# zhenghao2519/Beyond-Fixed-Forms

Measured on AMD Instinct MI355X. Metric: scenes/sec (2D->3D projection+refinement), 200k pts x 300 views, higher is better.
Workload: dtype f64

## Files before the change

beyond_fixed_forms_amd/_lib.py:

```python
from __future__ import annotations

import ctypes
import os
import time
from ctypes import c_double, c_float, c_int32, c_int64, c_void_p

import torch

_HERE = os.path.dirname(os.path.abspath(__file__))
LIB_PATH = os.environ.get("BFF_HIP_LIB") or os.path.join(_HERE, "lib", "libbff_hip.so")
CSRC_DIR = os.path.join(_HERE, "csrc")

_P, _I, _L, _D, _F = c_void_p, c_int32, c_int64, c_double, c_float

SIGNATURES = {
    "bff_rle_to_maskbits": [_P, _P, _P, _P, _I, _L, _I, _P, _P, _P],
    "bff_rle_to_labels": [_P, _P, _P, _P, _I, _L, _I, _P, _P, _P, _P],
    "bff_mask_row_directory": [_P, _P, _P, _I, _I, _I, _P, _P],
    "bff_project_views_lookup": [_P, _L, _L, _P, _P, _I, _P, _I, _I, _I, _P, _I, _I, _D, _P, _P, _P, _P, _P, _I, _P, _P, _P, _P, _P, _L, _L, _P, _P, _P, _P],
    "bff_project_views_cached": [_L, _I, _P, _I, _I, _P, _P, _P, _P, _P, _P, _P, _P, _I, _P, _P, _P, _P, _P, _L, _L, _P, _P, _P, _P],
    "bff_visibility_table": [_P, _L, _L, _P, _P, _I, _P, _I, _I, _I, _I, _I, _D, _P, _P, _P, _P, _L, _P, _I, _P],
    "bff_masks2d_count": [_P, _I, _L, _P, _P, _P],
    "bff_masks2d_runs": [_P, _I, _L, _P, _P, _P, _P],
    "bff_project_views": [_P, _L, _L, _P, _P, _I, _P, _P, _I, _I, _D, _P, _P, _P, _I, _P, _P, _P, _P, _P, _L, _L, _P, _P, _P, _P, _P],
    "bff_depth_tile_u16": [_P, _I, _I, _I, _P, _I, _P],
    "bff_project_views_u16": [_P, _L, _L, _P, _P, _I, _P, _I, _I, _I, _P, _I, _I, _D, _P, _P, _P, _I, _P, _P, _P, _P, _P, _L, _L, _P, _P, _P, _P, _P],
    "bff_point_tile_bounds": [_P, _L, _L, _P, _P],
    "bff_count_viewed": [_P, _L, _L, _P, _P, _I, _P, _I, _I, _I, _P, _I, _I, _D, _I, _P, _P, _P],
    "bff_render_depth_u16": [_P, _L, _L, _P, _P, _I, _I, _I, _I, _I, _I, _P, _P, _P, _P],
    "bff_render_splat_depth_u16": [_P, _L, _L, _P, _P, _I, _I, _I, _I, _I, _D, _I, _P, _P, _P, _P],
    "bff_point_labels": [_P, _I, _L, _L, _P, _P, _P],
    "bff_render_labels_u16": [_P, _L, _L, _P, _P, _P, _I, _I, _I, _I, _I, _D, _I, _P, _P, _P, _P, _P],
    "bff_label_runs_count": [_P, _I, _I, _I, _I, _I, _I, _P, _P, _P],
    "bff_label_runs_emit": [_P, _I, _I, _I, _I, _I, _I, _P, _L, _P, _P, _P, _P],
    "bff_render_mesh_depth_u16": [_P, _L, _L, _P, _L, _P, _P, _I, _I, _I, _I, _I, _I, _P, _P, _P],
    "bff_render_mesh_depth_clip_u16": [_P, _L, _L, _P, _L, _P, _P, _I, _I, _I, _I, _I, _D, _I, _P, _P, _P],
# ... 59 lines not shown
    "bff_dbscan_elements": [_P, _I, _L, _L, _P, _P, _P, _P, _P],
    "bff_dbscan_core": [_P, _I, _L, _P, _L, _P, _P, _P, _P, _L, _L, _P, _D, _D, _I, _P, _P],
    "bff_dbscan_link": [_P, _P, _P, _P, _I, _L, _P, _L, _P, _P, _P, _P, _L, _L, _P, _D, _D, _I, _P, _P],
}
PLAIN = {"bff_abi_version": (c_int32, []), "bff_last_error": (ctypes.c_char_p, []), "bff_arch": (ctypes.c_char_p, []),
         "bff_masks2d_tile_pixels": (c_int32, []), "bff_label_runs_tile_pixels": (c_int32, []), "bff_mask_lookup_rows": (c_int32, [c_int32, c_int32, c_int64]),
         "bff_cosine_gemm_path": (c_int32, [c_int32, c_int32, c_int32]),
         "bff_cross_popcount_slices": (c_int32, [c_int32, c_int32, c_int64]),
         "bff_chunk_mask_words": (c_int32, [c_int64]), "bff_label_plane_stride": (c_int64, [c_int64]), "bff_resolve_overlaps_max_rows": (c_int32, []),
         "bff_point_tile_size": (c_int32, []), "bff_sweep_frames_per_block": (c_int32, [c_int64, c_int32]), "bff_mesh_lane_box": (c_int32, []), "bff_splat_lane_box": (c_int32, []), "bff_depth_tiled_texels": (c_int64, [c_int32, c_int32]), "bff_merge_scratch_words": (c_int64, [c_int32]), "bff_merge_uses_chunk_bound": (c_int32, [c_int64]),
         "bff_profile_next_merge": (c_int32, [_P, _P]), "bff_group_slice_cap": (c_int32, [c_int32, c_int32]),
         "bff_point_threshold_scratch_words": (c_int64, [c_int64]), "bff_point_threshold_capacity": (c_int32, []), "bff_point_threshold_capacity_set": (c_int32, [c_int32]), "bff_scene_header_words": (c_int32, [c_int32, c_int32]), "bff_scene_struct_bytes": (c_int32, [c_int32]),
         "bff_host_component_csr": (c_int32, [_P, _P, _I, _I, _P, _P, _P, _P]),
         "bff_visibility_words": (c_int64, [c_int64]), "bff_visibility_builds": (c_int64, []),
         "bff_visibility_table_bytes": (c_int32, [c_int64, c_int32, c_int64, _P]),
         "bff_profile_next_sweep": (c_int32, [_P, _P]), "bff_event_create": (c_void_p, []),
         "bff_event_destroy": (c_int32, [_P]), "bff_event_elapsed_ms": (c_int32, [_P, _P, _P]),
         "bff_event_record": (c_int32, [_P, _P]), "bff_event_synchronize": (c_int32, [_P])}
ABI_VERSION = 16


class BffLibraryError(RuntimeError):
    pass


_lib = None


def load():
    global _lib
# ... 225 lines not shown


def visibility_builds():
    return int(load().bff_visibility_builds())


def visibility_table_bytes(n_points, n_slots, n_pixels=0):
    out = (c_int64 * 3)()
    rc = load().bff_visibility_table_bytes(n_points, n_slots, n_pixels, ctypes.cast(out, c_void_p))
    if rc != 0:
        raise RuntimeError(f"bff_visibility_table_bytes failed ({rc}): {load().bff_last_error().decode()}")
    return tuple(int(v) for v in out)


def visibility_table(xyz_soa, n_points, slot_inv_pose, cam_intr, depth, height, width, depth_thresh, tile_bounds=None,
                     depth_size=None, max_bytes=None):
    dev = xyz_soa.device
    n_slots = int(slot_inv_pose.shape[0])
    stride = visibility_words(n_points)
    hs, ws, layout = _depth_layout(depth, depth_size)
    if max_bytes is not None and sum(visibility_table_bytes(n_points, n_slots)) > max_bytes:
        return None
    mask = torch.empty((n_slots, stride), dtype=i64, device=dev)
    off = torch.empty((n_slots, stride), dtype=i32, device=dev)
    total = torch.zeros(1, dtype=i64, device=dev)
    head = (_ptr(xyz_soa, f64), n_points, xyz_soa.shape[1], _ptr(slot_inv_pose, f64), _k9(cam_intr), n_slots, _ptr(depth),
            hs, ws, layout, height, width, float(depth_thresh), _ptr(tile_bounds, f64), _ptr(mask, i64), _ptr(off, i32))
    call("bff_visibility_table", *head, None, 0, _ptr(total, i64), 1)
    n_pixels = int(total.item())
    if n_pixels >= 1 << 32 or (max_bytes is not None and sum(visibility_table_bytes(n_points, n_slots, n_pixels)) > max_bytes):
        return None
    pix = torch.empty(max(n_pixels, 1), dtype=i32, device=dev)
    call("bff_visibility_table", *head, _ptr(pix, i32), n_pixels, _ptr(total, i64), 2)
    return mask, off, pix


def project_views_cached(n_points, depth_index, height, width, vis, mask_tab, mask_dir, run_start, run_end, view_mask_offs,
                         word_bits, frame_mask, frame_rowbase, frame_nmask, frame_flags, rows, masked_count, viewed_count,
                         chunk_mask=None):
    call("bff_project_views_cached", n_points, depth_index.shape[0], _ptr(depth_index, i32), height, width,
         _ptr(vis[0], i64), _ptr(vis[1], i32), _ptr(vis[2], i32), _ptr(mask_tab, i32), _ptr(mask_dir, i32),
         _ptr(run_start, i32), _ptr(run_end, i32), _ptr(view_mask_offs, i32), word_bits, _ptr(frame_mask, i32),
         _ptr(frame_rowbase, i32), _ptr(frame_nmask, i32), _ptr(frame_flags, i32), _ptr(rows, i64),
         0 if rows is None else rows.shape[0], (n_points + 63) // 64, _ptr(chunk_mask, i64), _ptr(masked_count, i32),
         _ptr(viewed_count, i32))


def count_viewed(xyz_soa, n_points, inv_pose, cam_intr, depth, depth_index, height, width, depth_thresh, viewed_count,
                 tile_bounds=None, depth_size=None, frames_per_block=None):
    k = (c_double * 9)(*[float(v) for v in cam_intr.reshape(-1)])
    if depth.dtype == torch.int16 or depth_size is not None:
        hs, ws = (depth_size if depth_size is not None else depth.shape[1:3])
        layout = 0 if depth_size is None else (2 if depth.dtype == f32 else 1)
    else:
        hs, ws, layout = 0, 0, -1
        if depth.dtype != f32:
            raise TypeError(f"expected float32 depth images, got {depth.dtype}")
    if frames_per_block is None:
# ... 570 lines not shown
```

beyond_fixed_forms_amd/csrc/project.hip:

```cpp
#include <hip/hip_ext.h>

#include "common.h"
#include "mask_rows.h"

namespace bff {

constexpr int kBlock = 256;
constexpr int kPPT = 4;
constexpr int kWordsPerBlock = (kBlock / kWave) * kPPT;
constexpr int kPtsPerBlock = kWordsPerBlock * kWave;

struct Intrinsics { double k[9]; };

struct RawDepth {
    const uint32_t *taps;
    int n_taps;
    int texel_f32;
    int64_t frame_stride;
    float scale;
};

struct VisTable {
    const uint64_t *mask;
    const uint32_t *off;
// ... 728 lines not shown
    const int slot = blockIdx.y;
    if (w >= stride) return;
    const uint64_t m = mask[slot * stride + w];
    if (!((m >> lane) & 1)) return;
    const int64_t n = w * kWave + lane;
    const double px = xyz[n], py = xyz[n_pad + n], pz = xyz[2 * n_pad + n];
    const double *P = inv_pose + 16 * (int64_t)slot;
    const double cx = fma(P[3], 1.0, fma(P[2], pz, fma(P[1], py, fma(P[0], px, 0.0))));
    const double cy = fma(P[7], 1.0, fma(P[6], pz, fma(P[5], py, fma(P[4], px, 0.0))));
    const double cz = fma(P[11], 1.0, fma(P[10], pz, fma(P[9], py, fma(P[8], px, 0.0))));
    const double p0 = fma(K.k[2], cz, fma(K.k[1], cy, fma(K.k[0], cx, 0.0)));
    const double p1 = fma(K.k[5], cz, fma(K.k[4], cy, fma(K.k[3], cx, 0.0)));
    const double u = rint(p0 / cz), v = rint(p1 / cz);
    const int64_t at = (int64_t)off[slot * stride + w] + __popcll(m & ((1ull << lane) - 1));
    if (at < pix_cap) pixels[at] = (uint32_t)(int)u | ((uint32_t)(int)v << 16);
}

constexpr int kWaveChunk = 1024;
constexpr int kPx = kWaveChunk / kWave;
constexpr int kWaveChunks = 16384 / kWaveChunk;

__device__ __forceinline__ int chunk_word_slot(int i) { return i ^ ((((i >> 5) & 3) | ((i >> 4) & 8)) << 2); }

__device__ __forceinline__ uint32_t wave_xor_scan(uint32_t v)
{
#define BFF_DPP_XOR(ctrl, rows) v ^= (uint32_t)__builtin_amdgcn_update_dpp(0, (int)v, ctrl, rows, 0xF, false)
    BFF_DPP_XOR(0x111, 0xF);
    BFF_DPP_XOR(0x112, 0xF);
    BFF_DPP_XOR(0x114, 0xF);
    BFF_DPP_XOR(0x118, 0xF);
// ... 582 lines not shown
                                        int32_t word_bits, const int32_t *frame_mask, const int32_t *frame_rowbase,
                                        const int32_t *frame_nmask, const int32_t *frame_flags, uint64_t *rows, int64_t n_rows,
                                        int64_t nw, uint64_t *chunk_mask, int32_t *masked_count, int32_t *viewed_count,
                                        void *stream)
{
    if (n_points <= 0 || n_frames <= 0) return BFF_OK;
    BFF_REQUIRE(height > 0 && width > 0, "bff_project_views_cached: bad image size");
    BFF_REQUIRE(vis_mask && vis_off && vis_pix, "bff_project_views_cached: null table");
    const MaskRows mr{reinterpret_cast<const uint4 *>(mask_tab), mask_dir, run_start, run_end, view_mask_offs};
    const VisTable vt{vis_mask, vis_off, vis_pix, bff_visibility_words(n_points)};
    return project_views_launch(nullptr, n_points, n_points, nullptr, nullptr, n_frames, nullptr, nullptr, depth_index, height,
                                width, 0.0, nullptr, nullptr, nullptr, word_bits, frame_mask, frame_rowbase, frame_nmask,
                                frame_flags, rows, n_rows, nw, chunk_mask, masked_count, viewed_count, nullptr, stream, &mr, &vt);
}

extern "C" int64_t bff_visibility_words(int64_t n_points)
{
    return n_points <= 0 ? 0 : ceil_div(n_points, (int64_t)kPtsPerBlock) * kWordsPerBlock;
}

extern "C" int bff_visibility_table_bytes(int64_t n_points, int32_t n_slots, int64_t n_pixels, int64_t *bytes)
{
    BFF_REQUIRE(n_points >= 0 && n_slots >= 0 && n_pixels >= 0 && bytes, "bff_visibility_table_bytes: bad arguments");
    const int64_t entries = bff_visibility_words(n_points) * n_slots;
    bytes[0] = (int64_t)sizeof(uint64_t) * entries;
    bytes[1] = (int64_t)sizeof(uint32_t) * entries;
    bytes[2] = (int64_t)sizeof(uint32_t) * n_pixels;
    return BFF_OK;
}

// ... 124 lines not shown
```

beyond_fixed_forms_amd/csrc/scene.hip:

```cpp
#include "rows.h"

using namespace bff;

namespace {

__global__ void order_keys_kernel(const int64_t *__restrict__ sig, const int32_t *__restrict__ label_id, int n,
                                  int sig_bits, int64_t *__restrict__ keys)
{
    const int i = blockIdx.x * blockDim.x + threadIdx.x;
    if (i < n) keys[i] = ((int64_t)label_id[i] << sig_bits) | sig[i];
}

int bits_for(int n)
{
    int b = 1;
    while ((1 << b) < n && b < 31) ++b;
    return b;
}

}

#define BFF_TRY(call) do { const int rc_ = (call); if (rc_ != BFF_OK) return rc_; } while (0)

extern "C" int32_t bff_scene_header_words(int32_t s1_rows, int32_t cap)
// ... 53 lines not shown
    struct Prezeroed {
        Prezeroed() { scratch_prezeroed() = 1; }
        ~Prezeroed() { scratch_prezeroed() = 0; }
    } prezeroed_scope;
    void *hv = (ws->heavy_stream && ws->heavy_stream != stream) ? ws->heavy_stream : stream;
    const bool two = hv != stream;
    auto hand_over = [&](void *event, void *from, void *to) -> int {
        hipError_t ee = hipEventRecord(reinterpret_cast<hipEvent_t>(event), as_stream(from));
        if (ee == hipSuccess) ee = hipStreamWaitEvent(as_stream(to), reinterpret_cast<hipEvent_t>(event), 0);
        return ee == hipSuccess ? BFF_OK : fail((int)ee, "bff_scene_project: stream hand-over: %s", hipGetErrorString(ee));
    };
    if (two) {
        BFF_REQUIRE(ws->events[0] && ws->events[1] && ws->events[2] && ws->events[3], "bff_scene_project: a heavy stream needs the workspace's four events");
        BFF_TRY(hand_over(ws->events[0], stream, hv));
    }
    if (lookup) {
        BFF_REQUIRE(ws->mask_tab && ws->mask_dir, "bff_scene_project: no row directory buffers");
        BFF_TRY(bff_mask_row_directory(sc->run_start, sc->run_end, sc->mask_run_offs, n_rows, sc->height, sc->width,
                                       ws->mask_tab, ws->mask_dir, hv));
    } else {
        BFF_TRY(bff_rle_to_labels(sc->run_start, sc->run_end, sc->mask_run_offs, sc->view_mask_offs, sc->n_mviews, hw,
                                  sc->word_bits, ws->labels, ws->maskbits, ws->segmap, hv));
    }
    const bool ratio = pr->filter_mode == 2;
    int32_t *const sweep_viewed = (ratio && !viewed_in) ? ws->viewed : nullptr;
    const int32_t *const viewed = ratio ? (viewed_in ? viewed_in : ws->viewed) : nullptr;
    if (lookup && sc->vis_mask && sc->vis_off && sc->vis_pix)
        BFF_TRY(bff_project_views_cached(n, sc->n_frames, sc->depth_index, sc->height, sc->width, sc->vis_mask, sc->vis_off,
                                         sc->vis_pix, ws->mask_tab, ws->mask_dir, sc->run_start, sc->run_end,
                                         sc->view_mask_offs, sc->word_bits, sc->frame_mask, sc->frame_rowbase, sc->frame_nmask,
                                         sc->frame_flags, ws->rows, n_rows, nw, ws->chunk_mask, ws->masked, sweep_viewed, hv));
    else if (lookup)
        BFF_TRY(bff_project_views_lookup(sc->xyz, n, sc->n_pad, sc->inv_pose, sc->cam_intr, sc->n_frames,
                                         sc->depth_raw ? sc->depth_raw : (const void *)sc->depth, sc->depth_h, sc->depth_w,
                                         sc->depth_raw ? sc->depth_tiled : -1, sc->depth_index, sc->height, sc->width,
                                         pr->depth_thresh, ws->mask_tab, ws->mask_dir, sc->run_start, sc->run_end,
                                         sc->view_mask_offs, sc->word_bits, sc->frame_mask, sc->frame_rowbase, sc->frame_nmask,
                                         sc->frame_flags, ws->rows, n_rows, nw, ws->chunk_mask, ws->masked, sweep_viewed,
                                         sc->tile_bounds, hv));
    else if (sc->depth_raw)
        BFF_TRY(bff_project_views_u16(sc->xyz, n, sc->n_pad, sc->inv_pose, sc->cam_intr, sc->n_frames, sc->depth_raw,
                                      sc->depth_h, sc->depth_w, sc->depth_tiled, sc->depth_index, sc->height, sc->width, pr->depth_thresh,
// ... 87 lines not shown
```

beyond_fixed_forms_amd/pipeline.py:

```python
from __future__ import annotations

import ctypes
import os
import time
from ctypes import c_double, c_float, c_int32, c_int64, c_size_t, c_void_p

import numpy as np
import torch

from . import _lib

GROUP_CAP = 256
GROUP_CAP_MAX = 512
HDR_K, HDR_NUNIQUE, HDR_THR, HDR_OVERFLOW = 0, 4, 5, 6


def hdr_offsets(cap):
    return tuple(16 + k * cap for k in range(6))


class SceneStruct(ctypes.Structure):
    _fields_ = [("n_points", c_int64), ("n_pad", c_int64), ("nw", c_int64),
                ("xyz", c_void_p), ("tile_bounds", c_void_p), ("inv_pose", c_void_p), ("cam_intr", c_double * 9),
                ("depth", c_void_p), ("depth_raw", c_void_p),
                ("depth_index", c_void_p), ("frame_mask", c_void_p), ("frame_rowbase", c_void_p),
                ("frame_nmask", c_void_p), ("frame_flags", c_void_p),
                ("run_start", c_void_p), ("run_end", c_void_p), ("mask_run_offs", c_void_p), ("view_mask_offs", c_void_p),
                ("conf", c_void_p), ("label_id", c_void_p), ("unsort", c_void_p), ("perm", c_void_p),
                ("s1_run_start", c_void_p), ("s1_run_end", c_void_p), ("s1_row_run_offs", c_void_p),
                ("height", c_int32), ("width", c_int32), ("n_frames", c_int32), ("n_mviews", c_int32),
                ("word_bits", c_int32), ("n_rows", c_int32), ("conf_f16", c_int32), ("n_label_ids", c_int32),
                ("s1_rows", c_int32), ("depth_h", c_int32), ("depth_w", c_int32), ("depth_tiled", c_int32),
                ("vis_mask", c_void_p), ("vis_off", c_void_p), ("vis_pix", c_void_p)]


class ParamsStruct(ctypes.Structure):
    _fields_ = [("depth_thresh", c_double), ("filter_fraction", c_double), ("iou_thres", c_float),
                ("min_members", c_int32), ("filter_mode", c_int32), ("filter_sort", c_int32)]


_WS_PTRS = ["maskbits", "segmap", "labels", "rows", "chunk_mask", "keep", "tile_mask", "agg", "both",
            "masked", "viewed", "sel_scratch", "area", "mean_word", "order", "parent", "comp", "count",
            "gmembers", "goffs", "slices", "pair_scratch", "vals", "vals_sorted", "hist", "merge_scratch", "chunk_pop",
            "sig", "sig_keys", "sig_sorted", "sort_temp", "mask_tab", "mask_dir"]


class WorkspaceStruct(ctypes.Structure):
    _fields_ = [(n, c_void_p) for n in _WS_PTRS] + [("sort_temp_bytes", c_size_t), ("zero_bytes", c_size_t),
# ... 71 lines not shown
        setattr(s, k, _p(getattr(ds, k)))
    s.conf, s.unsort, s.perm = _p(ds.conf), _p(ds.unsort), _p(ds.perm)
    if ds.unsort is not None and ds.perm is None:
        raise ValueError("a spatially sorted scene needs its inverse permutation (DeviceScene.perm)")
    s.height, s.width = ds.height, ds.width
    s.n_frames = ds.n_frames if n_frames is None else n_frames
    s.n_mviews = ds.view_mask_offs.shape[0] - 1
    s.word_bits, s.n_rows = ds.word_bits, ds.n_rows
    s.conf_f16 = 1 if ds.conf.dtype == torch.float16 else 0
    s.n_label_ids = ds.n_label_ids
    if stage1 is not None:
        s.s1_run_start, s.s1_run_end, s.s1_row_run_offs = _p(stage1.run_start), _p(stage1.run_end), _p(stage1.row_run_offs)
        s.s1_rows = stage1.row_run_offs.shape[0] - 1
    if vis is not None:
        s.vis_mask, s.vis_off, s.vis_pix = _p(vis.mask), _p(vis.off), _p(vis.pix)
    return s


def params_struct(cfg, depth_thresh, filter_sort=False):
    _check_layout()
    p = ParamsStruct()
    from .scene import with_viewed_counts
    p.filter_sort = 1 if filter_sort else 0
    ratio = with_viewed_counts(cfg)
    p.depth_thresh = float(depth_thresh)
    p.filter_mode = 1 if cfg.if_occurance_threshold else (2 if ratio else 0)
    p.filter_fraction = float(cfg.detected_ratio_threshold if ratio else cfg.occurance_threshold)
    p.iou_thres = float(cfg.iou_thres)
    p.min_members = int(cfg.min_aggragated_masks)
    return p
# ... 309 lines not shown
```

beyond_fixed_forms_amd/projection.py:

```python
from __future__ import annotations

import dataclasses
from typing import List, Optional

import numpy as np
import torch

import os

from . import _lib, pipeline
from .scene import (DEPTH_THRESH, DeviceScene, prepare_class, prepare_geometry, prepare_scene,
                    with_viewed_counts)
from .timing import merge_span, span, sweep_span


@dataclasses.dataclass
class Stage2Result:
    scene_id: str
    n_points: int
    rows: torch.Tensor
    conf: torch.Tensor
    final_class: List[str]
    groups: list
    debug: dict
# ... 123 lines not shown
    stage1: Optional[object] = None


def fast_path_ok(ds: DeviceScene) -> bool:
    return (ds.n_rows > 0 and ds.n_points > 0 and ds.view_mask_offs.shape[0] > 1 and ds.n_mask_frames > 0
            and ds.xyz.is_cuda and os.environ.get("BFF_NO_FAST") != "1")


@dataclasses.dataclass
class VisibilityTable:
    mask: torch.Tensor
    off: torch.Tensor
    pix: torch.Tensor
    ready: torch.cuda.Event
    streams: set


def vis_table_max_bytes():
    return int(float(os.environ.get("BFF_VIS_TABLE_MAX_MB", "512")) * (1 << 20))


def scene_visibility(ds: DeviceScene, depth_thresh) -> Optional[VisibilityTable]:
    if os.environ.get("BFF_VIS_TABLE", "1") == "0" or not _lib.mask_lookup_rows(ds.height, ds.width, ds.n_rows):
        return None
    owner = ds.geometry if ds.geometry is not None else ds
    tables = owner.__dict__.setdefault("_vis_tables", {})
    key = float(depth_thresh)
    tab = tables.get(key)
    if tab is None:
        tables[key] = "visited"
        return None
    if tab is False:
        return None
    raw = _lib.raw_stream()
    if tab == "visited":
        dev = ds.xyz.device
        if ds.geometry is not None:
            poses = torch.as_tensor(np.ascontiguousarray(owner.inv_pose_host, dtype=np.float64).reshape(-1, 16)).to(dev)
        else:
            di = ds.depth_index.cpu().numpy()
            first = np.zeros(int(ds.sweep_depth.shape[0]), dtype=np.int64)
            slots, idx = np.unique(di, return_index=True)
            first[slots] = idx
            poses = ds.inv_pose[torch.as_tensor(first).to(dev)].contiguous()
        got = _lib.visibility_table(ds.xyz, ds.n_points, poses, ds.cam_intr, ds.sweep_depth, ds.height, ds.width, key,
                                    ds.tile_bounds, depth_size=ds.depth_size, max_bytes=vis_table_max_bytes())
        if got is None:
            tables[key] = False
            return None
        ready = torch.cuda.Event()
        ready.record(torch.cuda.current_stream(dev))
        tab = tables[key] = VisibilityTable(*got, ready=ready, streams={raw})
    elif raw not in tab.streams:
        st = torch.cuda.current_stream(ds.xyz.device)
        st.wait_event(tab.ready)
        for t in (tab.mask, tab.off, tab.pix):
            t.record_stream(st)
        tab.streams.add(raw)
    return tab


def projection_front(ds: DeviceScene, cfg, debug_out: bool = False, timers=None, stage1=None, fast=None) -> _Front:
    if fast is None:
        fast = not debug_out
    do_ratio = with_viewed_counts(cfg)
    viewed_in = ds.viewed_in if do_ratio else None
    if do_ratio and ds.geometry is not None and viewed_in is None:
        raise ValueError("a class scene needs its geometry's viewed counts for the detection-ratio filter "
                         "(prepare the geometry with with_viewed=True)")
    if fast and fast_path_ok(ds) and (stage1 is None or stage1.n_points == ds.n_points):
        fr = _Front(ds, cfg, {}, False, do_ratio=do_ratio, stage1=stage1)
        vis = scene_visibility(ds, DEPTH_THRESH)
        fr.dbg["sweep"] = "plain" if vis is None else "cached"
        with sweep_span(timers, "project_views"), merge_span(timers, "merge_components"):
            fr.fast = pipeline.issue(ds, cfg, DEPTH_THRESH, stage1,
                                     ds.n_frames if (do_ratio and viewed_in is None) else ds.n_mask_frames, viewed_in, vis)
        return fr
    with _lib.launch_stream():
        fr = _projection_front(ds, cfg, debug_out, timers, viewed_in=viewed_in)
        fr.stage1 = stage1
        return fr


def _projection_front(ds, cfg, debug_out, timers, viewed_in=None) -> _Front:
    dev = ds.xyz.device
    fr = _Front(ds, cfg, {}, debug_out)
    n, nw = ds.n_points, ds.nw
    do_ratio = fr.do_ratio = with_viewed_counts(cfg)
# ... 303 lines not shown
```

include/bff_hip.h:

```cpp
#ifndef BFF_HIP_H
#define BFF_HIP_H

#include <stddef.h>
#include <stdint.h>

#ifdef __cplusplus
extern "C" {
#endif

#define BFF_OK 0
#define BFF_E_ARG (-1)
#define BFF_E_LIMIT (-2)

#define BFF_ABI_VERSION 16

int bff_abi_version(void);
const char *bff_last_error(void);
const char *bff_arch(void);

int bff_host_component_csr(const int32_t *comp, const uint8_t *has_self_loop, int32_t n, int32_t min_members,
                           int32_t *offs, int32_t *members, int32_t *sizes, int32_t *n_void);

int bff_rle_to_maskbits(const int32_t *run_start, const int32_t *run_end, const int32_t *mask_run_offs,
                        const int32_t *view_mask_offs, int32_t n_views, int64_t n_pixels, int32_t word_bits,
// ... 232 lines not shown
int64_t bff_visibility_words(int64_t n_points);
int bff_visibility_table_bytes(int64_t n_points, int32_t n_slots, int64_t n_pixels, int64_t *bytes);
int bff_visibility_table(const double *xyz, int64_t n_points, int64_t n_pad, const double *slot_inv_pose,
                         const double *cam_intr_host, int32_t n_slots, const void *depth, int32_t depth_h,
                         int32_t depth_w, int32_t depth_layout, int32_t height, int32_t width, double depth_thresh,
                         const double *tile_bounds, uint64_t *vis_mask, uint32_t *vis_off, uint32_t *vis_pix,
                         int64_t pix_cap, uint64_t *n_pixels, int32_t phase, void *stream);
int64_t bff_visibility_builds(void);
int bff_project_views_cached(int64_t n_points, int32_t n_frames, const int32_t *depth_index, int32_t height,
                             int32_t width, const uint64_t *vis_mask, const uint32_t *vis_off, const uint32_t *vis_pix,
                             const uint32_t *mask_tab, const uint32_t *mask_dir, const int32_t *run_start,
                             const int32_t *run_end, const int32_t *view_mask_offs, int32_t word_bits,
                             const int32_t *frame_mask, const int32_t *frame_rowbase, const int32_t *frame_nmask,
                             const int32_t *frame_flags, uint64_t *rows, int64_t n_rows, int64_t nw, uint64_t *chunk_mask,
                             int32_t *masked_count, int32_t *viewed_count, void *stream);

typedef struct bff_scene {
    int64_t n_points, n_pad, nw;
    const double *xyz;
    const double *tile_bounds;
    const double *inv_pose;
    double cam_intr[9];
    const float *depth;
    const void *depth_raw;
    const int32_t *depth_index, *frame_mask, *frame_rowbase, *frame_nmask, *frame_flags;
    const int32_t *run_start, *run_end, *mask_run_offs, *view_mask_offs;
    const void *conf;
    const int32_t *label_id;
    const int32_t *unsort;
    const int32_t *perm;
    const int32_t *s1_run_start, *s1_run_end, *s1_row_run_offs;
    int32_t height, width, n_frames, n_mviews, word_bits, n_rows, conf_f16, n_label_ids, s1_rows, depth_h, depth_w,
            depth_tiled;
    const uint64_t *vis_mask;
    const uint32_t *vis_off, *vis_pix;
} bff_scene;

typedef struct bff_scene_params {
    double depth_thresh;
    double filter_fraction;
    float iou_thres;
    int32_t min_members;
    int32_t filter_mode;
    int32_t filter_sort;
} bff_scene_params;

typedef struct bff_scene_workspace {
    void *maskbits; uint32_t *segmap;
    uint8_t *labels;
    uint64_t *rows, *chunk_mask, *keep, *tile_mask, *agg, *both;
// ... 112 lines not shown
```

Before: 1422.

## Sweep projection by mask runs over a pixel-sorted visibility table

Adds a companion to the cached visibility table in which each slot's visible (pixel, point) pairs are radix-sorted by pixel, with per-row start offsets. A new runs sweep then binary-searches each RLE mask run's pixel range and sets the matching points' bits in an LDS row, instead of testing every visible point against a mask row directory. Separate count and viewed kernels replace the fused accounting. This removes the per-point directory lookup and the directory build, at the cost of extra memory, a one-time sort per table, and scattered shared-memory atomics.

```diff
diff --git a/beyond_fixed_forms_amd/_lib.py b/beyond_fixed_forms_amd/_lib.py
--- a/beyond_fixed_forms_amd/_lib.py
+++ b/beyond_fixed_forms_amd/_lib.py
@@ -20,6 +20,8 @@
     "bff_project_views_lookup": [_P, _L, _L, _P, _P, _I, _P, _I, _I, _I, _P, _I, _I, _D, _P, _P, _P, _P, _P, _I, _P, _P, _P, _P, _P, _L, _L, _P, _P, _P, _P],
     "bff_project_views_cached": [_L, _I, _P, _I, _I, _P, _P, _P, _P, _P, _P, _P, _P, _I, _P, _P, _P, _P, _P, _L, _L, _P, _P, _P, _P],
     "bff_visibility_table": [_P, _L, _L, _P, _P, _I, _P, _I, _I, _I, _I, _I, _D, _P, _P, _P, _P, _L, _P, _I, _P],
+    "bff_visibility_sorted": [_P, _P, _P, _L, _L, _I, _I, _I, _P, _P, _P, _P, _P, _P],
+    "bff_project_views_runs": [_L, _I, _P, _I, _I, _P, _P, _P, _P, _P, _P, _P, _P, _I, _P, _P, _P, _P, _P, _L, _L, _P, _P, _P, _P],
     "bff_masks2d_count": [_P, _I, _L, _P, _P, _P],
     "bff_masks2d_runs": [_P, _I, _L, _P, _P, _P, _P],
     "bff_project_views": [_P, _L, _L, _P, _P, _I, _P, _P, _I, _I, _D, _P, _P, _P, _I, _P, _P, _P, _P, _P, _L, _L, _P, _P, _P, _P, _P],
@@ -109,6 +111,8 @@
          "bff_host_component_csr": (c_int32, [_P, _P, _I, _I, _P, _P, _P, _P]),
          "bff_visibility_words": (c_int64, [c_int64]), "bff_visibility_builds": (c_int64, []),
          "bff_visibility_table_bytes": (c_int32, [c_int64, c_int32, c_int64, _P]),
+         "bff_visibility_sorted_bytes": (c_int32, [c_int32, c_int32, c_int64, _P]),
+         "bff_sweep_runs_ok": (c_int32, [c_int64]),
          "bff_profile_next_sweep": (c_int32, [_P, _P]), "bff_event_create": (c_void_p, []),
          "bff_event_destroy": (c_int32, [_P]), "bff_event_elapsed_ms": (c_int32, [_P, _P, _P]),
          "bff_event_record": (c_int32, [_P, _P]), "bff_event_synchronize": (c_int32, [_P])}
@@ -364,7 +368,7 @@
 
 
 def visibility_table(xyz_soa, n_points, slot_inv_pose, cam_intr, depth, height, width, depth_thresh, tile_bounds=None,
-                     depth_size=None, max_bytes=None):
+                     depth_size=None, max_bytes=None, with_count=False):
     dev = xyz_soa.device
     n_slots = int(slot_inv_pose.shape[0])
     stride = visibility_words(n_points)
@@ -382,7 +386,7 @@
         return None
     pix = torch.empty(max(n_pixels, 1), dtype=i32, device=dev)
     call("bff_visibility_table", *head, _ptr(pix, i32), n_pixels, _ptr(total, i64), 2)
-    return mask, off, pix
+    return (mask, off, pix, n_pixels) if with_count else (mask, off, pix)
 
 
 def project_views_cached(n_points, depth_index, height, width, vis, mask_tab, mask_dir, run_start, run_end, view_mask_offs,
@@ -392,6 +396,50 @@
          _ptr(vis[0], i64), _ptr(vis[1], i32), _ptr(vis[2], i32), _ptr(mask_tab, i32), _ptr(mask_dir, i32),
          _ptr(run_start, i32), _ptr(run_end, i32), _ptr(view_mask_offs, i32), word_bits, _ptr(frame_mask, i32),
          _ptr(frame_rowbase, i32), _ptr(frame_nmask, i32), _ptr(frame_flags, i32), _ptr(rows, i64),
+         0 if rows is None else rows.shape[0], (n_points + 63) // 64, _ptr(chunk_mask, i64), _ptr(masked_count, i32),
+         _ptr(viewed_count, i32))
+
+
+def visibility_sorted_bytes(n_slots, height, n_pixels=0):
+    out = (c_int64 * 3)()
+    rc = load().bff_visibility_sorted_bytes(n_slots, height, n_pixels, ctypes.cast(out, c_void_p))
+    if rc != 0:
+        raise RuntimeError(f"bff_visibility_sorted_bytes failed ({rc}): {load().bff_last_error().decode()}")
+    return tuple(int(v) for v in out)
+
+
+sorted_temp_bytes = 0
+
+
+def visibility_sorted(vis, n_pixels, n_points, height, width):
+    global sorted_temp_bytes
+    mask, off, pix = vis
+    dev = mask.device
+    n_slots = int(mask.shape[0])
+    spix = torch.empty(max(n_pixels, 1), dtype=i32, device=dev)
+    spt = torch.empty(max(n_pixels, 1), dtype=i32, device=dev)
+    rowstart = torch.zeros((n_slots, height + 1), dtype=i32, device=dev)
+    need = ctypes.c_size_t(0)
+    args = (n_pixels, n_points, n_slots, height, width)
+    call("bff_visibility_sorted", None, None, None, *args, None, None, None, None, ctypes.byref(need))
+    sorted_temp_bytes = int(need.value)
+    temp = torch.empty(max(int(need.value), 1), dtype=u8, device=dev)
+    call("bff_visibility_sorted", _ptr(mask, i64), _ptr(off, i32), _ptr(pix, i32), *args, _ptr(spix, i32), _ptr(spt, i32),
+         _ptr(rowstart, i32), _ptr(temp), ctypes.byref(need))
+    return spix, spt, rowstart
+
+
+def sweep_runs_ok(n_points):
+    return bool(load().bff_sweep_runs_ok(n_points))
+
+
+def project_views_runs(n_points, depth_index, height, width, vis, vis_sorted, run_start, run_end, mask_run_offs,
+                       view_mask_offs, word_bits, frame_mask, frame_rowbase, frame_nmask, frame_flags, rows, masked_count,
+                       viewed_count, chunk_mask):
+    call("bff_project_views_runs", n_points, depth_index.shape[0], _ptr(depth_index, i32), height, width,
+         _ptr(vis[0], i64), _ptr(vis_sorted[0], i32), _ptr(vis_sorted[1], i32), _ptr(vis_sorted[2], i32),
+         _ptr(run_start, i32), _ptr(run_end, i32), _ptr(mask_run_offs, i32), _ptr(view_mask_offs, i32), word_bits,
+         _ptr(frame_mask, i32), _ptr(frame_rowbase, i32), _ptr(frame_nmask, i32), _ptr(frame_flags, i32), _ptr(rows, i64),
          0 if rows is None else rows.shape[0], (n_points + 63) // 64, _ptr(chunk_mask, i64), _ptr(masked_count, i32),
          _ptr(viewed_count, i32))
 
diff --git a/beyond_fixed_forms_amd/csrc/project.hip b/beyond_fixed_forms_amd/csrc/project.hip
--- a/beyond_fixed_forms_amd/csrc/project.hip
+++ b/beyond_fixed_forms_amd/csrc/project.hip
@@ -1,4 +1,8 @@
+#include <algorithm>
+#include <cstdlib>
+
 #include <hip/hip_ext.h>
+#include <rocprim/device/device_radix_sort.hpp>
 
 #include "common.h"
 #include "mask_rows.h"
@@ -766,6 +770,242 @@
     const double u = rint(p0 / cz), v = rint(p1 / cz);
     const int64_t at = (int64_t)off[slot * stride + w] + __popcll(m & ((1ull << lane) - 1));
     if (at < pix_cap) pixels[at] = (uint32_t)(int)u | ((uint32_t)(int)v << 16);
+}
+
+
+__global__ __launch_bounds__(kBlock) void vis_sort_keys_kernel(const uint64_t *__restrict__ mask, const uint32_t *__restrict__ off,
+                                                               const uint32_t *__restrict__ pix, int64_t stride, int64_t n_pairs,
+                                                               int W, uint32_t hw, uint32_t *__restrict__ keys,
+                                                               uint32_t *__restrict__ pts)
+{
+    const int lane = threadIdx.x & 63;
+    const int64_t w = (int64_t)blockIdx.x * (kBlock / kWave) + (threadIdx.x >> 6);
+    const int slot = blockIdx.y;
+    if (w >= stride) return;
+    const uint64_t m = mask[slot * stride + w];
+    if (!((m >> lane) & 1)) return;
+    const int64_t at = (int64_t)off[slot * stride + w] + __popcll(m & ((1ull << lane) - 1));
+    if (at >= n_pairs) return;
+    const uint32_t p = pix[at];
+    keys[at] = (uint32_t)slot * hw + (p >> 16) * (uint32_t)W + (p & 0xffffu);
+    pts[at] = (uint32_t)(w * kWave + lane);
+}
+
+__global__ __launch_bounds__(kBlock) void vis_sorted_pixels_kernel(const uint32_t *__restrict__ keys, int64_t n_pairs, uint32_t hw,
+                                                                   uint32_t *__restrict__ spix)
+{
+    const int64_t i = (int64_t)blockIdx.x * kBlock + threadIdx.x;
+    if (i < n_pairs) spix[i] = keys[i] % hw;
+}
+
+__global__ __launch_bounds__(kBlock) void vis_rowstart_kernel(const uint32_t *__restrict__ spix, const uint32_t *__restrict__ off,
+                                                              int64_t stride, int64_t n_pairs, int n_slots, int H, int W,
+                                                              uint32_t *__restrict__ rowstart)
+{
+    const int64_t t = (int64_t)blockIdx.x * kBlock + threadIdx.x;
+    if (t >= (int64_t)n_slots * (H + 1)) return;
+    const int s = (int)(t / (H + 1)), y = (int)(t - (int64_t)s * (H + 1));
+    int64_t lo = min((int64_t)off[s * stride], n_pairs);
+    int64_t hi = s + 1 < n_slots ? min((int64_t)off[(s + 1) * stride], n_pairs) : n_pairs;
+    const uint32_t target = (uint32_t)y * (uint32_t)W;
+    while (lo < hi) {
+        const int64_t mid = lo + ((hi - lo) >> 1);
+        if (spix[mid] < target) lo = mid + 1; else hi = mid;
+    }
+    rowstart[t] = (uint32_t)lo;
+}
+
+constexpr int kRunsDeal = 4;
+
+__global__ __launch_bounds__(kBlock) void sweep_runs_fill_kernel(
+    int n_frames, const int32_t *__restrict__ depth_index, int H, int W,
+    const uint32_t *__restrict__ spix, const uint32_t *__restrict__ spt, const uint32_t *__restrict__ rowstart,
+    const int32_t *__restrict__ run_start, const int32_t *__restrict__ run_end, const int32_t *__restrict__ mask_run_offs,
+    const int32_t *__restrict__ view_mask_offs, const int32_t *__restrict__ frame_mask,
+    const int32_t *__restrict__ frame_rowbase, const int32_t *__restrict__ frame_nmask,
+    uint64_t *__restrict__ rows, int64_t nw, int n_chunks, uint64_t *__restrict__ chunk_mask, int mw)
+{
+    extern __shared__ uint64_t s_row[];
+    const int f = blockIdx.x, m = blockIdx.y;
+    const int mi = frame_mask[f];
+    if (mi < 0 || m >= frame_nmask[f]) return;
+    const int tid = threadIdx.x, lane = tid & 63, wave = tid >> 6;
+    const int64_t row = (int64_t)frame_rowbase[f] + m;
+    for (int i = tid; i < n_chunks * kCW; i += kBlock) s_row[i] = 0;
+    __syncthreads();
+
+    const int g = view_mask_offs[mi] + m;
+    const int r0 = mask_run_offs[g], r1 = mask_run_offs[g + 1];
+    const uint32_t *rs = rowstart + (int64_t)depth_index[f] * (H + 1);
+    const int hw = H * W;
+    uint32_t *bits = reinterpret_cast<uint32_t *>(s_row);
+    for (int rb = r0 + wave * kWave; rb < r1; rb += kBlock) {
+        const int r = rb + lane;
+        uint32_t lo = 0, cnt = 0;
+        if (r < r1) {
+            const int start = max(run_start[r], 0), end = min(run_end[r], hw);
+            if (start < end) {
+                const int y = start / W, ye = (end - 1) / W;
+                uint32_t lo1 = rs[y], hi1 = rs[y + 1], lo2 = rs[ye], hi2 = rs[ye + 1];
+                while (lo1 < hi1 || lo2 < hi2) {
+                    const bool go1 = lo1 < hi1, go2 = lo2 < hi2;
+                    const uint32_t mid1 = lo1 + ((hi1 - lo1) >> 1), mid2 = lo2 + ((hi2 - lo2) >> 1);
+                    const uint32_t v1 = go1 ? spix[mid1] : 0u, v2 = go2 ? spix[mid2] : 0u;
+                    if (go1) { if (v1 < (uint32_t)start) lo1 = mid1 + 1; else hi1 = mid1; }
+                    if (go2) { if (v2 < (uint32_t)end) lo2 = mid2 + 1; else hi2 = mid2; }
+                }
+                lo = lo1;
+                cnt = lo2 - lo1;
+            }
+        }
+        uint32_t incl = cnt;
+#pragma unroll
+        for (int d = 1; d < kWave; d <<= 1) {
+            const uint32_t t = __shfl_up(incl, d);
+            if (lane >= d) incl += t;
+        }
+        const uint32_t total = __shfl(incl, kWave - 1);
+        const uint32_t base = lo - (incl - cnt);
+        for (uint32_t k0 = 0; k0 < total; k0 += kRunsDeal * kWave) {
+            uint32_t at[kRunsDeal], pt[kRunsDeal];
+#pragma unroll
+            for (int j = 0; j < kRunsDeal; ++j) {
+                const uint32_t k = k0 + j * kWave + lane;
+                int owner = 0;
+#pragma unroll
+                for (int step = kWave / 2; step; step >>= 1)
+                    if (__shfl(incl, owner + step - 1) <= k) owner += step;
+                at[j] = __shfl(base, owner & (kWave - 1)) + k;
+            }
+#pragma unroll
+            for (int j = 0; j < kRunsDeal; ++j) pt[j] = k0 + j * kWave + lane < total ? spt[at[j]] : 0u;
+#pragma unroll
+            for (int j = 0; j < kRunsDeal; ++j)
+                if (k0 + j * kWave + lane < total) atomicOr(bits + (pt[j] >> 5), 1u << (pt[j] & 31));
+        }
+    }
+    __syncthreads();
+
+    for (int c0 = wave * kWave; c0 < n_chunks; c0 += kBlock) {
+        const int c = c0 + lane;
+        uint64_t v[kCW] = {};
+        if (c < n_chunks) {
+#pragma unroll
+            for (int q = 0; q < kCW; ++q) v[q] = s_row[c * kCW + q];
+        }
+        bool any = false;
+#pragma unroll
+        for (int h = 0; h < kCW; h += kPPT) {
+            uint64_t o = 0;
+#pragma unroll
+            for (int q = 0; q < kPPT; ++q) o |= v[h + q];
+            if (o) {
+                any = true;
+#pragma unroll
+                for (int q = 0; q < kPPT; ++q) {
+                    const int64_t w = (int64_t)c * kCW + h + q;
+                    if (w < nw) rows[row * nw + w] = v[h + q];
+                }
+            }
+        }
+        const uint64_t flags = __ballot(any);
+        if (lane == 0 && flags) chunk_mask[row * mw + (c0 >> 6)] |= flags;
+    }
+}
+
+constexpr int kCountBlock = 1024;
+constexpr int kCountBatch = 4;
+constexpr int kCountList = 4096;
+
+__global__ __launch_bounds__(kCountBlock) void sweep_runs_count_kernel(const uint64_t *__restrict__ rows, int64_t n_rows, int64_t nw,
+                                                                       const uint64_t *__restrict__ chunk_mask, int mw,
+                                                                       int64_t n_points, int32_t *__restrict__ masked_count)
+{
+    __shared__ int s_cnt[kCW * kWave];
+    __shared__ int s_list[kCountList];
+    __shared__ int s_n;
+    const int tid = threadIdx.x, lane = tid & 63, wave = tid >> 6;
+    const int c = blockIdx.x;
+    static_assert(kCountList == kCountBatch * kCountBlock, "a round lists what one batch of flag loads covers");
+    for (int i = tid; i < kCW * kWave; i += kCountBlock) s_cnt[i] = 0;
+    int cnt[8] = {};
+    const int64_t word = (int64_t)c * kCW + (lane >> 3);
+    const int shift = 8 * (lane & 7);
+    const uint64_t *flag = chunk_mask + (c >> 6);
+    for (int64_t r0 = 0; r0 < n_rows; r0 += kCountList) {
+        if (tid == 0) s_n = 0;
+        __syncthreads();
+        bool set[kCountBatch];
+#pragma unroll
+        for (int k = 0; k < kCountBatch; ++k) {
+            const int64_t r = r0 + k * kCountBlock + tid;
+            set[k] = r < n_rows && ((flag[r * mw] >> (c & 63)) & 1);
+        }
+#pragma unroll
+        for (int k = 0; k < kCountBatch; ++k)
+            if (set[k]) s_list[atomicAdd(&s_n, 1)] = k * kCountBlock + tid;
+        __syncthreads();
+        const int n = s_n;
+        for (int i0 = wave * kCountBatch; i0 < n; i0 += (kCountBlock / kWave) * kCountBatch) {
+            uint64_t v[kCountBatch];
+#pragma unroll
+            for (int k = 0; k < kCountBatch; ++k)
+                v[k] = (i0 + k < n && word < nw) ? rows[(r0 + s_list[i0 + k]) * nw + word] : 0;
+#pragma unroll
+            for (int k = 0; k < kCountBatch; ++k) {
+                const uint32_t b = (uint32_t)(v[k] >> shift) & 0xffu;
+#pragma unroll
+                for (int q = 0; q < 8; ++q) cnt[q] += (b >> q) & 1;
+            }
+        }
+        __syncthreads();
+    }
+#pragma unroll
+    for (int q = 0; q < 8; ++q)
+        if (cnt[q]) atomicAdd(&s_cnt[8 * lane + q], cnt[q]);
+    __syncthreads();
+    for (int i = tid; i < kCW * kWave; i += kCountBlock) {
+        const int64_t n = (int64_t)c * kCW * kWave + i;
+        if (n < n_points && s_cnt[i]) masked_count[n] += s_cnt[i];
+    }
+}
+
+constexpr int kViewedBatch = 4;
+
+__global__ __launch_bounds__(kBlock) void sweep_runs_viewed_kernel(int n_frames, const int32_t *__restrict__ depth_index,
+                                                                   const int32_t *__restrict__ frame_flags,
+                                                                   const uint64_t *__restrict__ vis_mask, int64_t stride,
+                                                                   int64_t nw, int64_t n_points, int32_t *__restrict__ viewed_count)
+{
+    const int lane = threadIdx.x & 63;
+    const int64_t w = (int64_t)blockIdx.x * (kBlock / kWave) + (threadIdx.x >> 6);
+    if (w >= nw) return;
+    int cnt = 0;
+    for (int f0 = 0; f0 < n_frames; f0 += kViewedBatch * kWave) {
+        uint64_t m[kViewedBatch];
+        int32_t slot[kViewedBatch], flags[kViewedBatch];
+#pragma unroll
+        for (int k = 0; k < kViewedBatch; ++k) {
+            const int f = f0 + k * kWave + lane;
+            slot[k] = f < n_frames ? depth_index[f] : 0;
+            flags[k] = f < n_frames ? frame_flags[f] : 0;
+        }
+#pragma unroll
+        for (int k = 0; k < kViewedBatch; ++k) m[k] = (flags[k] & 1) ? vis_mask[(int64_t)slot[k] * stride + w] : 0;
+#pragma unroll
+        for (int k = 0; k < kViewedBatch; ++k) {
+            uint64_t live = __ballot(m[k] != 0);
+            while (live) {
+                const int l = __ffsll((unsigned long long)live) - 1;
+                live &= live - 1;
+                const uint32_t lo = (uint32_t)__builtin_amdgcn_readlane((int)(uint32_t)m[k], l);
+                const uint32_t hi = (uint32_t)__builtin_amdgcn_readlane((int)(uint32_t)(m[k] >> 32), l);
+                cnt += (int)(((((uint64_t)hi << 32) | lo) >> lane) & 1);
+            }
+        }
+    }
+    const int64_t n = w * kWave + lane;
+    if (n < n_points && cnt) viewed_count[n] += cnt;
 }
 
 constexpr int kWaveChunk = 1024;
@@ -1378,6 +1618,111 @@
                                 frame_flags, rows, n_rows, nw, chunk_mask, masked_count, viewed_count, nullptr, stream, &mr, &vt);
 }
 
+constexpr int64_t kRunsLdsMax = 64 * 1024;
+
+static int64_t runs_row_bytes(int64_t n_points)
+{
+    return (int64_t)sizeof(uint64_t) * kCW * ceil_div(ceil_div(n_points, (int64_t)kWave), (int64_t)kCW);
+}
+
+extern "C" int32_t bff_sweep_runs_ok(int64_t n_points)
+{
+    const char *on = getenv("BFF_SWEEP_RUNS"), *cap = getenv("BFF_SWEEP_RUNS_LDS_BYTES");
+    if (on && on[0] == '0' && on[1] == 0) return 0;
+    int64_t bound = kRunsLdsMax;
+    if (cap && *cap) bound = std::min<int64_t>(bound, std::max<int64_t>(0, atoll(cap)));
+    return n_points > 0 && runs_row_bytes(n_points) <= bound;
+}
+
+extern "C" int bff_project_views_runs(int64_t n_points, int32_t n_frames, const int32_t *depth_index, int32_t height,
+                                      int32_t width, const uint64_t *vis_mask, const uint32_t *vis_spix,
+                                      const uint32_t *vis_spt, const uint32_t *vis_rowstart, const int32_t *run_start,
+                                      const int32_t *run_end, const int32_t *mask_run_offs, const int32_t *view_mask_offs,
+                                      int32_t word_bits, const int32_t *frame_mask, const int32_t *frame_rowbase,
+                                      const int32_t *frame_nmask, const int32_t *frame_flags, uint64_t *rows, int64_t n_rows,
+                                      int64_t nw, uint64_t *chunk_mask, int32_t *masked_count, int32_t *viewed_count,
+                                      void *stream)
+{
+    if (n_points <= 0 || n_frames <= 0) return BFF_OK;
+    BFF_REQUIRE(height > 0 && width > 0, "bff_project_views_runs: bad image size");
+    BFF_LIMIT((int64_t)height * width < (1ll << 31), "bff_project_views_runs: image larger than 2^31 pixels");
+    BFF_REQUIRE(vis_mask && vis_spix && vis_spt && vis_rowstart, "bff_project_views_runs: null table");
+    BFF_REQUIRE(word_bits == 32 || word_bits == 64, "bff_project_views_runs: word_bits must be 32 or 64");
+    BFF_REQUIRE(depth_index && frame_mask && frame_rowbase && frame_nmask && frame_flags && run_start && run_end &&
+                mask_run_offs && view_mask_offs && rows && chunk_mask && n_rows >= 0, "bff_project_views_runs: null pointer");
+    BFF_REQUIRE(nw == ceil_div(n_points, 64), "bff_project_views_runs: nw must be ceil(n_points/64)");
+    const int64_t row_bytes = runs_row_bytes(n_points);
+    BFF_LIMIT(row_bytes <= kRunsLdsMax, "bff_project_views_runs: an instance row exceeds 64 KB of LDS (bff_sweep_runs_ok)");
+    hipStream_t st = as_stream(stream);
+    const int n_chunks = (int)ceil_div(nw, kCW), mw = (int)ceil_div(n_chunks, 64);
+    const hipEvent_t ev0 = g_sweep_start, ev1 = g_sweep_stop;
+    g_sweep_start = g_sweep_stop = nullptr;
+    const bool count = masked_count != nullptr && n_rows > 0, viewed = viewed_count != nullptr;
+    hipExtLaunchKernelGGL(sweep_runs_fill_kernel, dim3((unsigned)n_frames, (unsigned)word_bits), dim3(kBlock),
+        (unsigned)row_bytes, st, ev0, (count || viewed) ? nullptr : ev1, 0,
+        n_frames, depth_index, height, width, vis_spix, vis_spt, vis_rowstart, run_start, run_end, mask_run_offs,
+        view_mask_offs, frame_mask, frame_rowbase, frame_nmask, rows, nw, n_chunks, chunk_mask, mw);
+    if (count)
+        hipExtLaunchKernelGGL(sweep_runs_count_kernel, dim3((unsigned)n_chunks), dim3(kCountBlock), 0, st,
+            nullptr, viewed ? nullptr : ev1, 0, rows, n_rows, nw, chunk_mask, mw, n_points, masked_count);
+    if (viewed)
+        hipExtLaunchKernelGGL(sweep_runs_viewed_kernel, dim3((unsigned)ceil_div(nw, kBlock / kWave)), dim3(kBlock), 0, st,
+            nullptr, ev1, 0, n_frames, depth_index, frame_flags, vis_mask, bff_visibility_words(n_points), nw, n_points,
+            viewed_count);
+    return launched("bff_project_views_runs");
+}
+
+extern "C" int bff_visibility_sorted_bytes(int32_t n_slots, int32_t height, int64_t n_pixels, int64_t *bytes)
+{
+    BFF_REQUIRE(n_slots >= 0 && height >= 0 && n_pixels >= 0 && bytes, "bff_visibility_sorted_bytes: bad arguments");
+    bytes[0] = (int64_t)sizeof(uint32_t) * n_pixels;
+    bytes[1] = (int64_t)sizeof(uint32_t) * n_pixels;
+    bytes[2] = (int64_t)sizeof(uint32_t) * n_slots * ((int64_t)height + 1);
+    return BFF_OK;
+}
+
+extern "C" int bff_visibility_sorted(const uint64_t *vis_mask, const uint32_t *vis_off, const uint32_t *vis_pix,
+                                     int64_t n_pixels, int64_t n_points, int32_t n_slots, int32_t height, int32_t width,
+                                     uint32_t *vis_spix, uint32_t *vis_spt, uint32_t *vis_rowstart, void *temp,
+                                     size_t *temp_bytes, void *stream)
+{
+    BFF_REQUIRE(n_pixels >= 0 && n_points >= 0 && n_slots >= 0 && temp_bytes, "bff_visibility_sorted: bad sizes");
+    BFF_REQUIRE(height > 0 && width > 0, "bff_visibility_sorted: bad image size");
+    BFF_LIMIT(height < (1 << 15) && width < (1 << 15), "bff_visibility_sorted: image too large for packed pixels");
+    BFF_LIMIT(n_slots <= 65535, "bff_visibility_sorted: too many depth slots");
+    BFF_LIMIT(n_pixels < (1ll << 32), "bff_visibility_sorted: more than 2^32 visible pairs");
+    const int64_t hw = (int64_t)height * width, span = hw * std::max(n_slots, 1);
+    BFF_LIMIT(span <= (1ll << 32), "bff_visibility_sorted: slots x pixels exceed the 32-bit sort key");
+    hipStream_t st = as_stream(stream);
+    unsigned key_bits = 1;
+    while (key_bits < 32 && (1ll << key_bits) < span) ++key_bits;
+    const size_t part = ((size_t)n_pixels * sizeof(uint32_t) + 255) & ~(size_t)255;
+    size_t need = 0;
+    hipError_t e = rocprim::radix_sort_pairs(nullptr, need, (const uint32_t *)nullptr, (uint32_t *)nullptr,
+                                             (const uint32_t *)nullptr, (uint32_t *)nullptr, (size_t)n_pixels, 0, key_bits, st);
+    if (e != hipSuccess) return fail((int)e, "bff_visibility_sorted: %s", hipGetErrorString(e));
+    if (!temp) { *temp_bytes = 3 * part + need; return BFF_OK; }
+    BFF_REQUIRE(*temp_bytes >= 3 * part + need, "bff_visibility_sorted: temp storage too small");
+    if (n_slots == 0 || n_points == 0) return BFF_OK;
+    BFF_REQUIRE(vis_mask && vis_off && vis_rowstart && (n_pixels == 0 || (vis_pix && vis_spix && vis_spt)),
+                "bff_visibility_sorted: null pointer");
+    const int64_t stride = bff_visibility_words(n_points);
+    if (n_pixels > 0) {
+        uint32_t *keys = reinterpret_cast<uint32_t *>(temp);
+        uint32_t *pts = reinterpret_cast<uint32_t *>(reinterpret_cast<char *>(temp) + part);
+        uint32_t *sorted = reinterpret_cast<uint32_t *>(reinterpret_cast<char *>(temp) + 2 * part);
+        dim3 grid((unsigned)ceil_div(stride, kBlock / kWave), (unsigned)n_slots);
+        vis_sort_keys_kernel<<<grid, kBlock, 0, st>>>(vis_mask, vis_off, vis_pix, stride, n_pixels, width, (uint32_t)hw, keys, pts);
+        e = rocprim::radix_sort_pairs(reinterpret_cast<char *>(temp) + 3 * part, need, (const uint32_t *)keys, sorted,
+                                      (const uint32_t *)pts, vis_spt, (size_t)n_pixels, 0, key_bits, st);
+        if (e != hipSuccess) return fail((int)e, "bff_visibility_sorted: %s", hipGetErrorString(e));
+        vis_sorted_pixels_kernel<<<(unsigned)ceil_div(n_pixels, kBlock), kBlock, 0, st>>>(sorted, n_pixels, (uint32_t)hw, vis_spix);
+    }
+    vis_rowstart_kernel<<<(unsigned)ceil_div((int64_t)n_slots * (height + 1), kBlock), kBlock, 0, st>>>(
+        vis_spix, vis_off, stride, n_pixels, n_slots, height, width, vis_rowstart);
+    return launched("bff_visibility_sorted");
+}
+
 extern "C" int64_t bff_visibility_words(int64_t n_points)
 {
     return n_points <= 0 ? 0 : ceil_div(n_points, (int64_t)kPtsPerBlock) * kWordsPerBlock;
diff --git a/beyond_fixed_forms_amd/csrc/scene.hip b/beyond_fixed_forms_amd/csrc/scene.hip
--- a/beyond_fixed_forms_amd/csrc/scene.hip
+++ b/beyond_fixed_forms_amd/csrc/scene.hip
@@ -91,18 +91,25 @@
         BFF_REQUIRE(ws->events[0] && ws->events[1] && ws->events[2] && ws->events[3], "bff_scene_project: a heavy stream needs the workspace's four events");
         BFF_TRY(hand_over(ws->events[0], stream, hv));
     }
-    if (lookup) {
+    const bool cached = lookup && sc->vis_mask && sc->vis_off && sc->vis_pix;
+    const bool runs = cached && sc->vis_spix && sc->vis_spt && sc->vis_rowstart && bff_sweep_runs_ok(n) != 0;
+    if (lookup && !runs) {
         BFF_REQUIRE(ws->mask_tab && ws->mask_dir, "bff_scene_project: no row directory buffers");
         BFF_TRY(bff_mask_row_directory(sc->run_start, sc->run_end, sc->mask_run_offs, n_rows, sc->height, sc->width,
                                        ws->mask_tab, ws->mask_dir, hv));
-    } else {
+    } else if (!lookup) {
         BFF_TRY(bff_rle_to_labels(sc->run_start, sc->run_end, sc->mask_run_offs, sc->view_mask_offs, sc->n_mviews, hw,
                                   sc->word_bits, ws->labels, ws->maskbits, ws->segmap, hv));
     }
     const bool ratio = pr->filter_mode == 2;
     int32_t *const sweep_viewed = (ratio && !viewed_in) ? ws->viewed : nullptr;
     const int32_t *const viewed = ratio ? (viewed_in ? viewed_in : ws->viewed) : nullptr;
-    if (lookup && sc->vis_mask && sc->vis_off && sc->vis_pix)
+    if (runs)
+        BFF_TRY(bff_project_views_runs(n, sc->n_frames, sc->depth_index, sc->height, sc->width, sc->vis_mask, sc->vis_spix,
+                                       sc->vis_spt, sc->vis_rowstart, sc->run_start, sc->run_end, sc->mask_run_offs,
+                                       sc->view_mask_offs, sc->word_bits, sc->frame_mask, sc->frame_rowbase, sc->frame_nmask,
+                                       sc->frame_flags, ws->rows, n_rows, nw, ws->chunk_mask, ws->masked, sweep_viewed, hv));
+    else if (cached)
         BFF_TRY(bff_project_views_cached(n, sc->n_frames, sc->depth_index, sc->height, sc->width, sc->vis_mask, sc->vis_off,
                                          sc->vis_pix, ws->mask_tab, ws->mask_dir, sc->run_start, sc->run_end,
                                          sc->view_mask_offs, sc->word_bits, sc->frame_mask, sc->frame_rowbase, sc->frame_nmask,
diff --git a/beyond_fixed_forms_amd/pipeline.py b/beyond_fixed_forms_amd/pipeline.py
--- a/beyond_fixed_forms_amd/pipeline.py
+++ b/beyond_fixed_forms_amd/pipeline.py
@@ -31,7 +31,8 @@
                 ("height", c_int32), ("width", c_int32), ("n_frames", c_int32), ("n_mviews", c_int32),
                 ("word_bits", c_int32), ("n_rows", c_int32), ("conf_f16", c_int32), ("n_label_ids", c_int32),
                 ("s1_rows", c_int32), ("depth_h", c_int32), ("depth_w", c_int32), ("depth_tiled", c_int32),
-                ("vis_mask", c_void_p), ("vis_off", c_void_p), ("vis_pix", c_void_p)]
+                ("vis_mask", c_void_p), ("vis_off", c_void_p), ("vis_pix", c_void_p),
+                ("vis_spix", c_void_p), ("vis_spt", c_void_p), ("vis_rowstart", c_void_p)]
 
 
 class ParamsStruct(ctypes.Structure):
@@ -133,6 +134,7 @@
         s.s1_rows = stage1.row_run_offs.shape[0] - 1
     if vis is not None:
         s.vis_mask, s.vis_off, s.vis_pix = _p(vis.mask), _p(vis.off), _p(vis.pix)
+        s.vis_spix, s.vis_spt, s.vis_rowstart = _p(vis.spix), _p(vis.spt), _p(vis.rowstart)
     return s
 
 
diff --git a/beyond_fixed_forms_amd/projection.py b/beyond_fixed_forms_amd/projection.py
--- a/beyond_fixed_forms_amd/projection.py
+++ b/beyond_fixed_forms_amd/projection.py
@@ -161,6 +161,12 @@
     pix: torch.Tensor
     ready: torch.cuda.Event
     streams: set
+    spix: Optional[torch.Tensor] = None
+    spt: Optional[torch.Tensor] = None
+    rowstart: Optional[torch.Tensor] = None
+
+    def tensors(self):
+        return [t for t in (self.mask, self.off, self.pix, self.spix, self.spt, self.rowstart) if t is not None]
 
 
 def vis_table_max_bytes():
@@ -191,17 +197,24 @@
             first[slots] = idx
             poses = ds.inv_pose[torch.as_tensor(first).to(dev)].contiguous()
         got = _lib.visibility_table(ds.xyz, ds.n_points, poses, ds.cam_intr, ds.sweep_depth, ds.height, ds.width, key,
-                                    ds.tile_bounds, depth_size=ds.depth_size, max_bytes=vis_table_max_bytes())
+                                    ds.tile_bounds, depth_size=ds.depth_size, max_bytes=vis_table_max_bytes(), with_count=True)
         if got is None:
             tables[key] = False
             return None
+        got, n_pairs = got[:3], got[3]
+        n_slots = int(got[0].shape[0])
+        total = sum(_lib.visibility_table_bytes(ds.n_points, n_slots, n_pairs)) + \
+            sum(_lib.visibility_sorted_bytes(n_slots, ds.height, n_pairs))
+        companion = (None, None, None)
+        if _lib.sweep_runs_ok(ds.n_points) and total <= vis_table_max_bytes() and n_slots * ds.height * ds.width <= 1 << 32:
+            companion = _lib.visibility_sorted(got, n_pairs, ds.n_points, ds.height, ds.width)
         ready = torch.cuda.Event()
         ready.record(torch.cuda.current_stream(dev))
-        tab = tables[key] = VisibilityTable(*got, ready=ready, streams={raw})
+        tab = tables[key] = VisibilityTable(*got, ready, {raw}, *companion)
     elif raw not in tab.streams:
         st = torch.cuda.current_stream(ds.xyz.device)
         st.wait_event(tab.ready)
-        for t in (tab.mask, tab.off, tab.pix):
+        for t in tab.tensors():
             t.record_stream(st)
         tab.streams.add(raw)
     return tab
@@ -219,6 +232,8 @@
         fr = _Front(ds, cfg, {}, False, do_ratio=do_ratio, stage1=stage1)
         vis = scene_visibility(ds, DEPTH_THRESH)
         fr.dbg["sweep"] = "plain" if vis is None else "cached"
+        if vis is not None:
+            fr.dbg["sweep_form"] = "runs" if vis.spix is not None and _lib.sweep_runs_ok(ds.n_points) else "points"
         with sweep_span(timers, "project_views"), merge_span(timers, "merge_components"):
             fr.fast = pipeline.issue(ds, cfg, DEPTH_THRESH, stage1,
                                      ds.n_frames if (do_ratio and viewed_in is None) else ds.n_mask_frames, viewed_in, vis)
diff --git a/include/bff_hip.h b/include/bff_hip.h
--- a/include/bff_hip.h
+++ b/include/bff_hip.h
@@ -270,6 +270,20 @@
                              const int32_t *frame_mask, const int32_t *frame_rowbase, const int32_t *frame_nmask,
                              const int32_t *frame_flags, uint64_t *rows, int64_t n_rows, int64_t nw, uint64_t *chunk_mask,
                              int32_t *masked_count, int32_t *viewed_count, void *stream);
+
+int bff_visibility_sorted(const uint64_t *vis_mask, const uint32_t *vis_off, const uint32_t *vis_pix, int64_t n_pixels,
+                          int64_t n_points, int32_t n_slots, int32_t height, int32_t width, uint32_t *vis_spix,
+                          uint32_t *vis_spt, uint32_t *vis_rowstart, void *temp, size_t *temp_bytes, void *stream);
+int bff_visibility_sorted_bytes(int32_t n_slots, int32_t height, int64_t n_pixels, int64_t *bytes);
+
+int32_t bff_sweep_runs_ok(int64_t n_points);
+int bff_project_views_runs(int64_t n_points, int32_t n_frames, const int32_t *depth_index, int32_t height, int32_t width,
+                           const uint64_t *vis_mask, const uint32_t *vis_spix, const uint32_t *vis_spt,
+                           const uint32_t *vis_rowstart, const int32_t *run_start, const int32_t *run_end,
+                           const int32_t *mask_run_offs, const int32_t *view_mask_offs, int32_t word_bits,
+                           const int32_t *frame_mask, const int32_t *frame_rowbase, const int32_t *frame_nmask,
+                           const int32_t *frame_flags, uint64_t *rows, int64_t n_rows, int64_t nw, uint64_t *chunk_mask,
+                           int32_t *masked_count, int32_t *viewed_count, void *stream);
 
 typedef struct bff_scene {
     int64_t n_points, n_pad, nw;
@@ -290,6 +304,7 @@
             depth_tiled;
     const uint64_t *vis_mask;
     const uint32_t *vis_off, *vis_pix;
+    const uint32_t *vis_spix, *vis_spt, *vis_rowstart;
 } bff_scene;
 
 typedef struct bff_scene_params {
```

New measurement: 1522, median of 6. +7.0%, better.
